# lorenzsp/EMRI_FrequencyDomainWaveforms

Hardware: AMD Instinct MI355X
Metric: FD waveforms/sec (2 yr, dt=10 s, ~3000 modes) at 1/2/4/8 GPUs; mode-sum HBM GB/s (higher is better)
Workload: dtype f64

## Files before the change

### emri_frequencydomainwaveforms_amd/csrc/emrifd.hip

```cpp

#include "emrifd_layout.h"

#define EFD_VERSION 100

static thread_local std::string g_err;

int efdhip::fail(int code, const std::string& msg) {
    g_err = msg;
    return code;
}

namespace {

constexpr int NWAVE = TILE / 64;
constexpr int XCD_GROUP = 1024 / TILE;
constexpr int SEGWIN = TILE;
constexpr int PIECES = (int)sizeof(Item) / 16;
constexpr int B_PIECE = (int)offsetof(Item, b) / 16;
constexpr int ROUNDS = 2;
constexpr int NC = (ROUNDS * TILE) / PIECES;


__device__ __forceinline__ bool seg_hits_tile(int2 lh, int32_t tlo, int32_t thi) {
    return lh.y > tlo && lh.x < thi;
// ... 1063 lines not shown
#pragma clang fp contract(off)
                    const int64_t q = j - k0, nb = nf - k0;
                    const double2 d0 = reinterpret_cast<const double2*>(lld)[q];
                    const double2 d1 = reinterpret_cast<const double2*>(lld)[nb + q];
                    const double w0 = llw[q], w1 = llw[nb + q];
                    const double r0 = d0.x - vp.x * w0, i0 = d0.y - vp.y * w0;
                    const double r1 = d1.x - vc.x * w1, i1 = d1.y - vc.y * w1;
                    llacc = fma(r0, r0, fma(i0, i0, llacc));
                    llacc = fma(r1, r1, fma(i1, i1, llacc));
                }
                if (!php) return;
                if (accumulate_out) {
                    const double2 pp = php[j - k0], pc = phc[j - k0];
                    vp.x += pp.x; vp.y += pp.y; vc.x += pc.x; vc.y += pc.y;
                }
                php[j - k0] = vp;
                phc[j - k0] = vc;
            };
            put(km, sm, sk);
            if (km != k) put(k, sk, sm);
        }
    }
    if constexpr (EPI == EPI_DH) {
        if (PAIRED && lld) {
            __shared__ double dhw4[3][NWAVE];
#pragma unroll
            for (int s = 0; s < 3; ++s) {
#pragma unroll
                for (int o = 32; o > 0; o >>= 1) dh[s] += __shfl_xor(dh[s], o, 64);
                if (lane == 0) dhw4[s][wave] = dh[s];
            }
            __syncthreads();
            if (tid < 3) {
                double t = 0.0;
#pragma unroll
                for (int w = 0; w < NWAVE; ++w) t += dhw4[tid][w];
                llpart[tid * ntiles + tile] = t;
            }
        }
    } else if (PAIRED && lld) {
#pragma unroll
        for (int o = 32; o > 0; o >>= 1) llacc += __shfl_xor(llacc, o, 64);
        __shared__ double llw4[NWAVE];
        if (lane == 0) llw4[wave] = llacc;
        __syncthreads();
        if (tid == 0) {
            double t = 0.0;
#pragma unroll
            for (int w = 0; w < NWAVE; ++w) t += llw4[w];
            llpart[tile] = t;
        }
    }
}

struct SumDesc {
    const Item* items;
    const int4* ranges;
    const int2* seglh;
    const int4* seginfo;
    const int32_t* nseg;
    const double* freq;
    const int32_t* gm;
    const int32_t* gn;
    const double* t;
    const double* coefA;
    const double* coefT;
    const double2* sctab;
    const uint32_t* tkeys;
    const int32_t* tcnt;
    const int32_t* tperm;
    const int32_t* segbase;
    const int32_t* stb0;
    const int32_t* stb1;
    Header* hdr;
    double* out;
    double* hp;
    double* hc;
    double* llpart;
    int64_t k0;
    int32_t nt, K;
};
template <bool PAIRED, int CAUSTIC, int NB = BPL, int EPI = EPI_LL>
__device__ __forceinline__ void modesum_tile(
    const SumDesc d, int64_t nf, int64_t nlanes, int64_t ntiles, int accumulate_out,
    const double* __restrict__ lld, const double* __restrict__ llw,
    const double* __restrict__ llconst, int64_t b, bool direct = false, int ioff = 0,
    double* __restrict__ spart = nullptr, int32_t* __restrict__ scnt = nullptr) {
    modesum_tile<PAIRED, CAUSTIC, NB, EPI>(
        d.items, d.ranges, d.seglh, d.seginfo, d.nseg, d.freq, nf, nlanes, ntiles, d.nt, d.K,
        d.gm, d.gn, d.t, d.coefA, d.coefT, d.sctab, d.tkeys, d.tcnt, d.tperm, d.segbase, d.stb0,
        d.stb1, d.hdr, accumulate_out, d.out, d.hp, d.hc, d.k0, lld, llw, d.llpart, llconst, b,
        direct, ioff, spart, scnt);
}

template <bool PAIRED, int CAUSTIC, int BPL>
__global__ __launch_bounds__(TILE) __attribute__((amdgpu_waves_per_eu(EFD_WAVES_PER_EU, 8)))
void k_modesum(const SumDesc d, int64_t nf, int64_t nlanes, int64_t ntiles, int accumulate_out) {
    modesum_tile<PAIRED, CAUSTIC>(d, nf, nlanes, ntiles, accumulate_out, nullptr, nullptr,
                                  nullptr, (int64_t)blockIdx.x);
}

struct SumBatch {
    SumDesc d[EFD_BATCH_MAX];
    int32_t n;
};
static_assert(sizeof(SumBatch) <= 3584, "batch descriptors must fit the kernel arguments");
template <class Outside>
__device__ __forceinline__ void ll_final_reduce(const double* __restrict__ p,
                                                const Header* __restrict__ h, bool sparse,
                                                Outside outside, int64_t ntiles, double scale,
                                                double* __restrict__ out) {
    __shared__ double red[256];
    int64_t t0 = 0, t1 = ntiles - 1;
    if (sparse) {
        const int32_t lo = h->lane_lo, hi = h->lane_hi;
        t0 = lo < hi ? lo / TILE_LANES : ntiles;
        t1 = lo < hi ? (int64_t)(hi - 1) / TILE_LANES : -1;
    }
    auto val = [&](int64_t i) { return (i < t0 || i > t1) ? outside(i) : p[i]; };
    double acc = 0.0;
    int64_t i = threadIdx.x;
    for (; i + 3 * 256 < ntiles; i += 4 * 256) {
        const double v0 = val(i), v1 = val(i + 256), v2 = val(i + 512), v3 = val(i + 768);
        acc += v0;
        acc += v1;
        acc += v2;
        acc += v3;
    }
    for (; i < ntiles; i += 256) acc += val(i);
    red[threadIdx.x] = acc;
    __syncthreads();
    for (int s = 128; s > 0; s >>= 1) {
        if ((int)threadIdx.x < s) red[threadIdx.x] += red[threadIdx.x + s];
        __syncthreads();
    }
    if (threadIdx.x == 0) {
        const bool bad = h->runs_overflow | h->bad_mn | h->bad_tile;
        *out = bad ? __longlong_as_double(0x7ff8000000000000LL) : scale * red[0];
    }
}
template <bool PAIRED, int CAUSTIC, int BPL, bool SPARSE, int EPI = EPI_LL>
__global__ __launch_bounds__(TILE) __attribute__((amdgpu_waves_per_eu(EFD_WAVES_PER_EU, 8)))
void k_modesum_batch(const SumBatch batch, int64_t nf, int64_t nlanes, int64_t ntiles,
                     int accumulate_out, const double* __restrict__ lld,
                     const double* __restrict__ llw, const double* __restrict__ llconst,
                     int64_t nper) {
    const int n = batch.n;
    int w;
    int64_t pos;
    if (lld == nullptr) {
        w = (int)(blockIdx.x % (unsigned)n);
        pos = blockIdx.x / (unsigned)n;
    } else {
        const unsigned g = blockIdx.x, r = g >> 3;
        w = (int)(r % (unsigned)n);
        pos = (int64_t)(r / (unsigned)n) * 8 + (g & 7u);
    }
    const SumDesc& d = batch.d[w];
    if constexpr (SPARSE) {
        const int32_t nit = d.hdr->nitems;
        if (nit > 0) {
            const Layout L = make_layout(d.nt, d.K, nf, 1);
            char* W = reinterpret_cast<char*>(d.hdr);
            const int4* items = ws_at<const int4>(W, L.sitem);
            for (int64_t it = pos; it < nit; it += nper) {
                const int4 e = items[it];
                const int S = e.y & 0xffff, j = e.y >> 16;
                if (S > 1)
                    modesum_tile<PAIRED, CAUSTIC, 1, EPI>(
                        d, nf, nlanes, ntiles, accumulate_out, lld, llw, llconst, e.x, true, j,
                        ws_at<double>(W, L.spart) + (size_t)e.z * TILE_LANES * 4,
                        ws_at<int32_t>(W, L.scnt) + e.w);
                else
                    modesum_tile<PAIRED, CAUSTIC, BPL, EPI>(d, nf, nlanes, ntiles, accumulate_out,
                                                            lld, llw, llconst, e.x, true);
                __syncthreads();
            }
            return;
        }
        const int32_t lo = d.hdr->lane_lo, hi = d.hdr->lane_hi;
        if (lo < hi) {
            const int64_t t1 = min((int64_t)(hi - 1) / TILE_LANES, ntiles - 1);
            for (int64_t tile = lo / TILE_LANES + pos; tile <= t1; tile += nper) {
                modesum_tile<PAIRED, CAUSTIC, BPL, EPI>(d, nf, nlanes, ntiles, accumulate_out, lld,
                                                        llw, llconst, tile, true);
                __syncthreads();
            }
        }
        return;
    }
    modesum_tile<PAIRED, CAUSTIC, BPL, EPI>(d, nf, nlanes, ntiles, accumulate_out, lld, llw,
                                            llconst, pos);
}

template <int BPL>
__global__ __launch_bounds__(TILE) void k_ll_tile_const(const double* __restrict__ lld,
                                                        const double* __restrict__ llw,
                                                        int64_t nf, int64_t nlanes, int64_t k0,
                                                        double* __restrict__ llconst) {
    const int64_t tile = blockIdx.x;
    __builtin_amdgcn_s_setreg(1 | (6 << 6) | (1 << 11), 0);
    __builtin_amdgcn_s_setreg(1 | (9 << 6), 0);
    const int tid = threadIdx.x;
    const int lane = tid & 63;
    const int wave = __builtin_amdgcn_readfirstlane(tid >> 6);
    const int32_t w_lo = (int32_t)(tile * TILE_LANES + wave * 64 * BPL);
    double llacc = 0.0;
#pragma unroll
    for (int i = 0; i < BPL; ++i) {
        const int64_t k = w_lo + 64 * i + lane;
        if (k >= nlanes) continue;
        const int64_t km = nf - 1 - k;
        double2 sk = make_double2(0.0, 0.0);
        double2 sm = make_double2(0.0, 0.0);
        if (km == k) {
            sk.x += sm.x;
            sk.y += sm.y;
            sm = sk;
        }
        auto put = [&](int64_t j, double2 a, double2 b) {
            if (j < k0) return;
            double2 vp = make_double2(0.5 * (a.x + b.x), 0.5 * (a.y - b.y));
            double2 vc = make_double2(-0.5 * (a.y + b.y), 0.5 * (a.x - b.x));
            {
#pragma clang fp contract(off)
                const int64_t q = j - k0, nb = nf - k0;
                const double2 d0 = reinterpret_cast<const double2*>(lld)[q];
                const double2 d1 = reinterpret_cast<const double2*>(lld)[nb + q];
                const double w0 = llw[q], w1 = llw[nb + q];
                const double r0 = d0.x - vp.x * w0, i0 = d0.y - vp.y * w0;
                const double r1 = d1.x - vc.x * w1, i1 = d1.y - vc.y * w1;
                llacc = fma(r0, r0, fma(i0, i0, llacc));
                llacc = fma(r1, r1, fma(i1, i1, llacc));
            }
        };
        put(km, sm, sk);
        if (km != k) put(k, sk, sm);
    }
#pragma unroll
    for (int o = 32; o > 0; o >>= 1) llacc += __shfl_xor(llacc, o, 64);
    __shared__ double llw4[NWAVE];
    if (lane == 0) llw4[wave] = llacc;
    __syncthreads();
    if (tid == 0) {
        double t = 0.0;
#pragma unroll
        for (int w = 0; w < NWAVE; ++w) t += llw4[w];
        llconst[tile] = t;
    }
}

struct LlBatch {
    const double* part[EFD_BATCH_MAX];
    const Header* hdr[EFD_BATCH_MAX];
    double* out;
    const double* llconst;
    int64_t ntiles;
    int32_t n;
};
struct StatusBatch {
    Header* h[EFD_BATCH_MAX];
    int32_t n;
};
__global__ __launch_bounds__(64) void k_lane_gather(const StatusBatch sb, int32_t* out) {
    const int i = threadIdx.x;
    if (i >= sb.n) return;
    out[2 * i] = sb.h[i]->lane_lo;
    out[2 * i + 1] = sb.h[i]->lane_hi;
}
__global__ __launch_bounds__(64) void k_status_gather(const StatusBatch sb, int32_t* out) {
    const int i = threadIdx.x;
    if (i >= sb.n) return;
    Header* h = sb.h[i];
    const int32_t f = (h->runs_overflow ? 1 : 0) | (h->bad_mn ? 2 : 0) | (h->bad_tile ? 4 : 0);
    out[i] = f;
    if (f) {
        h->runs_overflow = 0;
        h->bad_mn = 0;
        h->bad_tile = 0;
    }
}

__global__ __launch_bounds__(256) void k_ll_final(const LlBatch lb) {
    const double* llconst = lb.llconst;
    ll_final_reduce(lb.part[blockIdx.x], lb.hdr[blockIdx.x], llconst != nullptr,
                    [=](int64_t i) { return llconst[i]; }, lb.ntiles, -0.5 * 4.0,
                    lb.out + blockIdx.x);
}

struct DhBatch {
    const Header* hdr[EFD_BATCH_MAX];
    const double* part;
    double* out;
    int64_t ntiles;
    int32_t sparse;
};
__global__ __launch_bounds__(256) void k_dh_final(const DhBatch db) {
    const int64_t o = 3 * (int64_t)blockIdx.x + blockIdx.y;
    ll_final_reduce(db.part + o * db.ntiles, db.hdr[blockIdx.x], db.sparse != 0,
                    [](int64_t) { return 0.0; }, db.ntiles, 4.0, db.out + o);
}

constexpr int TK_HITS = TILE;
constexpr int TK_ROWS = 8;
__device__ __forceinline__ void tile_keys_body(
    const int4* __restrict__ ranges, const int2* __restrict__ seglh,
    const int4* __restrict__ seginfo, const int32_t* __restrict__ nsegp,
    const int32_t* __restrict__ segbase, const int32_t* __restrict__ stb0,
    const int32_t* __restrict__ stb1, int64_t ntiles, uint32_t* __restrict__ tkeys,
    int32_t* __restrict__ tcnt) {
    static_assert(SEGWIN == TILE, "one segment per thread and window row");
    __shared__ int hits[TK_HITS], hp0[TK_HITS], hcnt[TK_HITS], hoff[TK_HITS], hws[TK_HITS],
        hwt[TK_HITS];
    __shared__ int4 hinfo[TK_HITS];
    __shared__ int wcnt[TK_ROWS * NWAVE];
    __shared__ int part[NWAVE];
    const int64_t tile = blockIdx.x;
    if (tile >= ntiles) return;
    const int tid = threadIdx.x, lane = tid & 63;
    const int wave = __builtin_amdgcn_readfirstlane(tid >> 6);
    const int32_t tlo = (int32_t)(tile * TILE_LANES), thi = tlo + TILE_LANES;
    const int nseg = *nsegp;
    EFD_EXP_DO(if (tile == 0 && tid == 0) exp_add(27, (unsigned long long)nseg);)
    int nhit = 0;
    for (int base = 0; base < nseg; base += TK_ROWS * TILE) {
        unsigned long long bal[TK_ROWS];
#pragma unroll
        for (int r = 0; r < TK_ROWS; ++r) {
            const int sgi = base + r * TILE + tid;
            bool hit = false;
            if (sgi < nseg) hit = seg_hits_tile(seglh[sgi], tlo, thi);
            bal[r] = __ballot(hit);
            if (lane == 0) wcnt[r * NWAVE + wave] = __popcll(bal[r]);
        }
        __syncthreads();
#pragma unroll
        for (int r = 0; r < TK_ROWS; ++r) {
            int before = nhit;
            for (int w = 0; w < wave; ++w) before += wcnt[r * NWAVE + w];
            if ((bal[r] >> lane) & 1ull) {
                const int pos = before + __popcll(bal[r] & ((1ull << lane) - 1ull));
                if (pos < TK_HITS) hits[pos] = base + r * TILE + tid;
            }
#pragma unroll
            for (int w = 0; w < NWAVE; ++w) nhit += wcnt[r * NWAVE + w];
        }
        __syncthreads();
    }
    EFD_EXP_DO(if (tid == 0) exp_add(28, (unsigned long long)nhit);)
    if (nhit > TK_HITS) {
        if (tid == 0) tcnt[tile] = -1;
        return;
    }
    int c = 0;
    if (tid < nhit) {
        const int sg = hits[tid];
        const HitRecords hr = hit_records(sg, tile, tlo, thi, segbase, stb0, stb1, seginfo, ranges);
        c = hr.count;
        hp0[tid] = hr.p0;
        hcnt[tid] = c;
        hinfo[tid] = seginfo[sg];
    }
    int total;
    const int off = block_excl_scan<NWAVE>(c, part, lane, wave, total);
    if (total > KEYCAP) {
        if (tid == 0) tcnt[tile] = -1;
        return;
    }
    if (tid < nhit) hoff[tid] = off;
    __syncthreads();
    {
        const int w = tid < nhit ? hits[tid] / SEGWIN : INT32_MAX;
        const bool first = tid < nhit && (tid == 0 || hits[tid - 1] / SEGWIN != w);
        const bool last = tid < nhit && (tid == nhit - 1 || hits[tid + 1] / SEGWIN != w);
        int st = first ? off : INT32_MIN;
        int en = last ? off + c : INT32_MAX;
#pragma unroll
        for (int o = 1; o < 64; o <<= 1) {
            const int vs = __shfl_up(st, o, 64), ve = __shfl_down(en, o, 64);
            if (lane >= o) st = max(st, vs);
            if (lane + o < 64) en = min(en, ve);
        }
        if (lane == 63) hws[wave] = st;
        if (lane == 0) hwt[wave] = en;
        __syncthreads();
        for (int v = 0; v < wave; ++v) st = max(st, hws[v]);
        for (int v = NWAVE - 1; v > wave; --v) en = min(en, hwt[v]);
        __syncthreads();
        if (tid < nhit) {
            hws[tid] = st;
            hwt[tid] = en - st;
        }
    }
    __syncthreads();
    uint32_t* out = tkeys + (size_t)tile * KEYCAP;
    for (int g = tid; g < total; g += TILE) {
        int lo = 0, hi = nhit - 1;
        while (lo < hi) {
            const int mid = (lo + hi + 1) >> 1;
            if (hoff[mid] <= g) lo = mid; else hi = mid - 1;
        }
        const int ws = hws[lo], take = hwt[lo];
        out[ws + scatter_slot(g - ws, take)] = list_key(hinfo[lo], hp0[lo] + (g - hoff[lo]));
    }
    if (tid == 0) tcnt[tile] = total;
}
__global__ __launch_bounds__(TILE) void k_tile_keys(const PrepBatch B) {
    PREP_WALKER(B);
    if (D.lists == 0) return;
    tile_keys_body(ws_at<int4>(W, L.ranges), ws_at<int2>(W, L.seglh), ws_at<int4>(W, L.seginfo),
                   ws_at<int32_t>(W, L.nseg), ws_at<int32_t>(W, L.segbase),
                   ws_at<int32_t>(W, L.stb0), ws_at<int32_t>(W, L.stb1), L.ntiles,
                   ws_at<uint32_t>(W, L.tkeys), ws_at<int32_t>(W, L.tcnt));
}

constexpr int ORDER_BUCKETS = 64;
__device__ __forceinline__ int tile_cost_bucket(int32_t c) {
    if (c < 0) return ORDER_BUCKETS - 1;
    const float l = __log2f((float)c + 1.0f) * 4.0f;
    return min((int)l, ORDER_BUCKETS - 2);
}
__device__ __forceinline__ int wave_bucket_add(int* hist, int bucket, bool valid) {
    const int lane = threadIdx.x & 63;
    unsigned long long todo = __ballot(valid);
    int res = 0;
    while (todo) {
        const int leader = __ffsll((long long)todo) - 1;
        const int bl = __shfl(bucket, leader, 64);
        const unsigned long long same = __ballot(valid && bucket == bl) & todo;
        int base = 0;
        if (lane == leader) base = atomicAdd(&hist[bl], __popcll(same));
        base = __shfl(base, leader, 64);
        if ((same >> lane) & 1ull) res = base + __popcll(same & ((1ull << lane) - 1ull));
        todo &= ~same;
    }
    return res;
}
__device__ __forceinline__ void tile_order_body(const int32_t* __restrict__ tcnt,
                                                int64_t ntiles, int32_t* __restrict__ tperm) {
    __shared__ int hist[ORDER_BUCKETS];
    const int tid = threadIdx.x;
    if (tid < ORDER_BUCKETS) hist[tid] = 0;
    __syncthreads();
    constexpr int PER = 16;
    int bk[PER];
#pragma unroll
    for (int q = 0; q < PER; ++q) {
        const int64_t i = tid + (int64_t)q * 1024;
        bk[q] = i < ntiles ? tile_cost_bucket(tcnt[i]) : -1;
    }
#pragma unroll
    for (int q = 0; q < PER; ++q) wave_bucket_add(hist, bk[q], bk[q] >= 0);
    const int64_t npass = (ntiles + 1023) / 1024;
    for (int64_t p = PER; p < npass; ++p) {
        const int64_t i = tid + p * 1024;
        const int bkt = i < ntiles ? tile_cost_bucket(tcnt[i]) : 0;
        wave_bucket_add(hist, bkt, i < ntiles);
    }
    __syncthreads();
    if (tid == 0) {
        int acc = 0;
        for (int q = ORDER_BUCKETS - 1; q >= 0; --q) { const int h = hist[q]; hist[q] = acc; acc += h; }
    }
    __syncthreads();
#pragma unroll
    for (int q = 0; q < PER; ++q) {
        const int pos = wave_bucket_add(hist, bk[q], bk[q] >= 0);
        if (bk[q] >= 0) tperm[pos] = (int32_t)(tid + q * 1024);
    }
    for (int64_t p = PER; p < npass; ++p) {
        const int64_t i = tid + p * 1024;
        const int bkt = i < ntiles ? tile_cost_bucket(tcnt[i]) : 0;
        const int pos = wave_bucket_add(hist, bkt, i < ntiles);
        if (i < ntiles) tperm[pos] = (int32_t)i;
    }
}
__global__ __launch_bounds__(1024) void k_tile_order(const PrepBatch B) {
    PREP_WALKER(B);
    if (D.lists != 3) return;
    tile_order_body(ws_at<int32_t>(W, L.tcnt), L.ntiles, ws_at<int32_t>(W, L.tperm));
}

constexpr int TD_THREADS = 256;
constexpr int TD_SPL = 4;

__device__ __forceinline__ int knot_interval(const double* __restrict__ t, int nt, double x) {
    int lo = 0, hi = nt - 1;
    while (hi - lo > 1) {
        const int mid = (lo + hi) >> 1;
        if (t[mid] <= x) lo = mid; else hi = mid;
    }
    return lo;
}

template <bool WIN>
__global__ __launch_bounds__(TD_THREADS) void k_td_modesum(
    const double* __restrict__ t, int nt, const double* __restrict__ coefT,
    const double* __restrict__ coefA, const int32_t* __restrict__ gm,
    const int32_t* __restrict__ gn, int K, const Header* __restrict__ hdr, double dt,
    int64_t ns, int accumulate_out, double* __restrict__ out, double* __restrict__ hp,
    double* __restrict__ hc, const double* __restrict__ window) {
    const int64_t s_base = (int64_t)blockIdx.x * (TD_THREADS * TD_SPL) + threadIdx.x;
    const double t_end = t[nt - 1];
    const int G = hdr->groups;
    double w[TD_SPL], pphi[TD_SPL], pr[TD_SPL], zr[TD_SPL], zi[TD_SPL];
    int jj[TD_SPL];
    bool valid[TD_SPL];
    bool any_valid = false;
#pragma unroll
    for (int i = 0; i < TD_SPL; ++i) {
        const int64_t s = s_base + (int64_t)i * TD_THREADS;
        const double ts = (double)s * dt;
        valid[i] = s < ns && ts <= t_end;
        any_valid |= valid[i];
        jj[i] = valid[i] ? knot_interval(t, nt, ts) : nt - 2;
        w[i] = valid[i] ? ts - t[jj[i]] : 0.0;
        const double* ct = coefT + (size_t)jj[i] * 32;
        pphi[i] = fma(fma(fma(ct[0], w[i], ct[8]), w[i], ct[16]), w[i], ct[24]);
        pr[i] = fma(fma(fma(ct[1], w[i], ct[9]), w[i], ct[17]), w[i], ct[25]);
        double sn, cs;
        sincos_big(pr[i], sn, cs);
        zr[i] = cs;
        zi[i] = -sn;
    }
    double Hr[TD_SPL], Hi[TD_SPL];
#pragma unroll
    for (int i = 0; i < TD_SPL; ++i) Hr[i] = Hi[i] = 0.0;

    if (__any(any_valid) && G > 0) {
        const int j0 = (int)rfl((uint32_t)jj[0]);
        bool same = true;
#pragma unroll
        for (int i = 0; i < TD_SPL; ++i) same &= jj[i] == j0;
        const size_t row = (size_t)4 * 4 * K;
        auto run = [&](auto UNI) {
            constexpr bool U = decltype(UNI)::value;
            double Pr[TD_SPL], Pi[TD_SPL], Qr[TD_SPL], Qi[TD_SPL];
#pragma unroll
            for (int i = 0; i < TD_SPL; ++i) Pr[i] = Pi[i] = Qr[i] = Qi[i] = 0.0;
            auto flush = [&](int m, int n0) {
#pragma unroll
                for (int i = 0; i < TD_SPL; ++i) {
                    double sn, cs;
                    sincos_big(fma((double)m, pphi[i], (double)n0 * pr[i]), sn, cs);
                    const double br = cs, bi = -sn;
                    Hr[i] += (br * Pr[i] - bi * Pi[i]) + (br * Qr[i] - bi * Qi[i]);
                    Hi[i] += (br * Pi[i] + bi * Pr[i]) - (br * Qi[i] + bi * Qr[i]);
                    Pr[i] = Pi[i] = Qr[i] = Qi[i] = 0.0;
                }
            };
            int cur_m = gm[G - 1], nprev = gn[G - 1];
            for (int g = G - 1; g >= 0; --g) {
                const int m = gm[g], n = gn[g];
                int d = nprev - n;
                if (m != cur_m) {
                    flush(cur_m, nprev);
                    cur_m = m;
                    d = 1;
                }
                nprev = n;
                for (; d > 1; --d) {
#pragma unroll
                    for (int i = 0; i < TD_SPL; ++i) {
                        const double a = Pr[i], b = Qr[i];
                        Pr[i] = fma(a, zr[i], -Pi[i] * zi[i]);
                        Pi[i] = fma(a, zi[i], Pi[i] * zr[i]);
                        Qr[i] = fma(b, zr[i], -Qi[i] * zi[i]);
                        Qi[i] = fma(b, zi[i], Qi[i] * zr[i]);
                    }
                }
#pragma unroll
                for (int i = 0; i < TD_SPL; ++i) {
                    const double* ca = coefA + (size_t)(U ? j0 : jj[i]) * row + 4 * g;
                    const double wi = w[i];
                    const double bpr = fma(fma(fma(ca[0], wi, ca[4 * K]), wi, ca[8 * K]), wi, ca[12 * K]);
                    const double bpi = fma(fma(fma(ca[1], wi, ca[4 * K + 1]), wi, ca[8 * K + 1]), wi, ca[12 * K + 1]);
                    const double bmr = fma(fma(fma(ca[2], wi, ca[4 * K + 2]), wi, ca[8 * K + 2]), wi, ca[12 * K + 2]);
                    const double bmi = fma(fma(fma(ca[3], wi, ca[4 * K + 3]), wi, ca[8 * K + 3]), wi, ca[12 * K + 3]);
                    const double a = Pr[i], b = Qr[i];
                    Pr[i] = fma(a, zr[i], fma(-Pi[i], zi[i], bpr));
                    Pi[i] = fma(a, zi[i], fma(Pi[i], zr[i], bpi));
                    Qr[i] = fma(b, zr[i], fma(-Qi[i], zi[i], bmr));
                    Qi[i] = fma(b, zi[i], fma(Qi[i], zr[i], bmi));
                }
            }
            flush(cur_m, nprev);
        };
        if (__all(same)) run(std::integral_constant<bool, true>{});
        else run(std::integral_constant<bool, false>{});
    }

    double2* o = reinterpret_cast<double2*>(out);
#pragma unroll
    for (int i = 0; i < TD_SPL; ++i) {
        const int64_t s = s_base + (int64_t)i * TD_THREADS;
        if (s >= ns) continue;
        double vr = valid[i] ? -Hr[i] : 0.0, vi = valid[i] ? -Hi[i] : 0.0;
        if constexpr (WIN) {
            const double wv = window[s];
            vr *= wv;
            vi *= wv;
        }
        if (o) {
            double2 v = make_double2(vr, vi);
            if (accumulate_out) { const double2 p = o[s]; v.x += p.x; v.y += p.y; }
            o[s] = v;
        }
        if (hp) hp[s] = accumulate_out ? hp[s] + vr : vr;
        if (hc) hc[s] = accumulate_out ? hc[s] - vi : -vi;
    }
}

}


static int64_t resident_tile_slots() {
    constexpr int MAX_DEV = 64;
    static std::atomic<int64_t> cache[MAX_DEV];
    int dev = 0;
    if (hipGetDevice(&dev) != hipSuccess || dev < 0 || dev >= MAX_DEV) return 1024;
    int64_t v = cache[dev].load(std::memory_order_relaxed);
    if (v > 0) return v;
    int cus = 0, per_cu = 0;
    if (hipDeviceGetAttribute(&cus, hipDeviceAttributeMultiprocessorCount, dev) != hipSuccess ||
        hipOccupancyMaxActiveBlocksPerMultiprocessor(
            &per_cu, reinterpret_cast<const void*>(&k_modesum<true, EFD_CAUSTIC_UNIFORM, BPL>),
            TILE, 0) != hipSuccess || cus <= 0 || per_cu <= 0)
        return 1024;
    v = (int64_t)cus * per_cu;
    cache[dev].store(v, std::memory_order_relaxed);
    return v;
}

constexpr int32_t ORDER_MIN_K = 1024;
constexpr int32_t LISTS_MIN_K = 1024;
static int32_t lists_min_k() {
    static const int32_t v = [] {
        const char* e = std::getenv("EFD_LISTS_MIN_K");
        return e ? (int32_t)std::atoi(e) : LISTS_MIN_K;
    }();
    return v;
}
static bool use_prebuilt(int32_t K) { return K >= lists_min_k(); }
static bool use_cost_order(int64_t ntiles, int32_t K) {
    return use_prebuilt(K) && K >= ORDER_MIN_K && ntiles > resident_tile_slots();
}
int32_t efdhip::list_mode(int32_t K, int64_t ntiles) {
    return use_prebuilt(K) ? (use_cost_order(ntiles, K) ? 3 : 1) : 0;
}

int efdhip::check_modesum_args(const efd_modesum_args* a, const void* workspace, int phase) {
    if (!a || !workspace) return fail(EFD_ERR_ARG, "efd_modesum: NULL argument");
    if (!a->t || !a->phi_phi || !a->phi_r || !a->f_phi || !a->f_r || !a->amp || !a->m ||
        !a->n || !a->ylm_p || !a->ylm_m || !a->freq)
        return fail(EFD_ERR_ARG, "efd_modesum: NULL array");
    const bool pol = a->hp != nullptr || a->hc != nullptr;
    if (pol && (!a->hp || !a->hc || !a->grid_symmetric || a->k0 < 0 || a->k0 > a->nf))
        return fail(EFD_ERR_ARG, "efd_modesum: hp/hc need both pointers, a symmetric grid and "
                                 "0 <= k0 <= nf");
    if ((phase & 2) && !a->out && !pol)
        return fail(EFD_ERR_ARG, "efd_modesum: no output (out or hp/hc)");
    if (a->nt < 2 || a->nt > MAX_NT) return fail(EFD_ERR_ARG, "efd_modesum: nt out of range");
    if (a->K <= 0 || a->K > MAX_K) return fail(EFD_ERR_ARG, "efd_modesum: K out of range [1, 8192]");
    if (a->nf <= 0 || a->nf >= (int64_t)INT32_MAX)
        return fail(EFD_ERR_ARG, "efd_modesum: nf out of range");
    if (a->caustic != EFD_CAUSTIC_SPA && a->caustic != EFD_CAUSTIC_UNIFORM)
        return fail(EFD_ERR_ARG, "efd_modesum: unknown caustic mode");
    return EFD_OK;
}

int efdhip::launch_tile_lists(const void* prep_batch, int64_t ntiles, bool any_lists,
                              bool any_order, hipStream_t st) {
    const PrepBatch& B = *static_cast<const PrepBatch*>(prep_batch);
    const unsigned nz = (unsigned)B.n;
    if (any_lists) {
        hipLaunchKernelGGL(k_tile_keys, dim3((unsigned)ntiles, 1, nz), dim3(TILE), 0, st, B);
        HIP_TRY(hipGetLastError());
    }
    if (any_order) {
        hipLaunchKernelGGL(k_tile_order, dim3(1, 1, nz), dim3(1024), 0, st, B);
        HIP_TRY(hipGetLastError());
    }
    return EFD_OK;
}

static SumDesc sum_desc(const efd_modesum_args* a, void* workspace, const Layout& L) {
    char* ws = (char*)workspace;
    const int32_t lists = efdhip::list_mode(a->K, L.ntiles);
    SumDesc d{};
    d.items = (const Item*)(ws + L.items);
    d.ranges = (const int4*)(ws + L.ranges);
    d.seglh = (const int2*)(ws + L.seglh);
    d.seginfo = (const int4*)(ws + L.seginfo);
    d.nseg = (const int32_t*)(ws + L.nseg);
    d.freq = a->freq;
    d.gm = (const int32_t*)(ws + L.gm);
    d.gn = (const int32_t*)(ws + L.gn);
    d.t = a->t;
    d.coefA = (const double*)(ws + L.coefA);
    d.coefT = (const double*)(ws + L.coefT);
    d.sctab = (const double2*)(ws + L.sctab);
    d.tkeys = (const uint32_t*)(ws + L.tkeys);
    d.tcnt = lists ? (const int32_t*)(ws + L.tcnt) : nullptr;
    d.tperm = lists == 3 ? (const int32_t*)(ws + L.tperm) : nullptr;
    d.segbase = (const int32_t*)(ws + L.segbase);
    d.stb0 = (const int32_t*)(ws + L.stb0);
    d.stb1 = (const int32_t*)(ws + L.stb1);
    d.hdr = (Header*)(ws + L.header);
    d.out = a->out;
    d.hp = a->hp;
    d.hc = a->hc;
    d.llpart = (double*)(ws + L.llpart);
    d.k0 = a->k0;
    d.nt = a->nt;
    d.K = a->K;
    return d;
}

template <class F>
static void for_sum_variant(bool paired, int caustic, F f) {
    using Uniform = std::integral_constant<int, EFD_CAUSTIC_UNIFORM>;
    using Spa = std::integral_constant<int, EFD_CAUSTIC_SPA>;
    if (paired) {
        if (caustic == EFD_CAUSTIC_UNIFORM) f(std::true_type{}, Uniform{});
        else f(std::true_type{}, Spa{});
    } else {
        if (caustic == EFD_CAUSTIC_UNIFORM) f(std::false_type{}, Uniform{});
        else f(std::false_type{}, Spa{});
    }
}

static int read_header(const void* workspace, void* stream, Header& h) {
    HIP_TRY(hipStreamSynchronize((hipStream_t)stream));
    HIP_TRY(hipMemcpy(&h, workspace, sizeof(Header), hipMemcpyDeviceToHost));
    return EFD_OK;
}

static int fill_status_batch(const char* fn, void* const* workspace, int32_t count,
                             StatusBatch& sb) {
    sb.n = count;
    for (int i = 0; i < count; ++i) {
        if (!workspace[i]) return fail(EFD_ERR_ARG, std::string(fn) + ": NULL workspace");
        sb.h[i] = (Header*)workspace[i];
    }
    return EFD_OK;
}

static int status_error(int32_t flags, const std::string& who) {
    if (flags & 1) return fail(EFD_ERR_ARG, who + "a harmonic has more than 8 monotonic runs");
    if (flags & 2) return fail(EFD_ERR_ARG, who + "|m| > 255 or |n| > 1023");
    return fail(EFD_ERR_HIP, who + "a tile dispatch-order entry was out of range (prepare/sum "
                                   "workspace mismatch?); bins were left unwritten");
}

extern "C" {

int efd_version(void) { return EFD_VERSION; }

#ifndef EFD_BUILD_ID
#define EFD_BUILD_ID "unversioned"
#endif
__attribute__((used)) static const char efd_build_tag[] = "EFD_BUILD_ID=" EFD_BUILD_ID;
const char* efd_build_id(void) { return efd_build_tag + 13; }

#ifdef EFD_EXP
int efd_exp_counters(unsigned long long* out) {
    HIP_TRY(hipDeviceSynchronize());
    HIP_TRY(hipMemcpyFromSymbol(out, HIP_SYMBOL(g_exp_count), sizeof(unsigned long long) * EXP_NCOUNT));
    return EFD_OK;
}
int efd_exp_tiles(unsigned int* out, unsigned long long* clk) {
    HIP_TRY(hipDeviceSynchronize());
    HIP_TRY(hipMemcpyFromSymbol(out, HIP_SYMBOL(g_exp_tile), sizeof(unsigned int) * 16384));
    HIP_TRY(hipMemcpyFromSymbol(clk, HIP_SYMBOL(g_exp_tclk), sizeof(unsigned long long) * 16384));
    return EFD_OK;
}
#endif

int efd_last_error(char* buf, int len) {
    if (!buf || len <= 0) return EFD_ERR_ARG;
    std::snprintf(buf, (size_t)len, "%s", g_err.c_str());
    return EFD_OK;
}

size_t efd_modesum_workspace_bytes(int32_t nt, int32_t K, int64_t nf) {
    if (nt < 2 || nt > MAX_NT || K <= 0 || K > MAX_K || nf <= 0) return 0;
    return make_layout(nt, K, nf, 0).total;
}

static int modesum_impl(const efd_modesum_args* a, void* workspace, size_t workspace_bytes,
                        void* stream, int phase) {
    {
        const int rc = efdhip::check_modesum_args(a, workspace, phase);
        if (rc != EFD_OK) return rc;
    }
    const int paired = a->grid_symmetric ? 1 : 0;
    const Layout L = make_layout(a->nt, a->K, a->nf, paired);
    if (workspace_bytes < L.total)
        return fail(EFD_ERR_WORKSPACE, "efd_modesum: workspace too small (see efd_modesum_workspace_bytes)");

    hipStream_t st = (hipStream_t)stream;
    if (phase & 1) {
        const int rc = efdhip::prepare_batch("efd_modesum_prepare", &a, &workspace,
                                             &workspace_bytes, 1, stream);
        if (rc != EFD_OK) return rc;
    }
    if (phase & 2) {
        const int64_t gq = 8 * XCD_GROUP;
        const dim3 grid((unsigned)((L.ntiles + gq - 1) / gq * gq)), block(TILE);
        const int acc = a->accumulate ? 1 : 0;
        const SumDesc d = sum_desc(a, workspace, L);
        if (a->prof_begin) HIP_TRY(hipEventRecord((hipEvent_t)a->prof_begin, st));
        for_sum_variant(paired != 0, a->caustic, [&](auto P, auto C) {
            hipLaunchKernelGGL((k_modesum<decltype(P)::value, decltype(C)::value, BPL>), grid,
                               block, 0, st, d, a->nf, L.nlanes, L.ntiles, acc);
        });
        HIP_TRY(hipGetLastError());
        if (a->prof_end) HIP_TRY(hipEventRecord((hipEvent_t)a->prof_end, st));
    }
    return EFD_OK;
}

int efd_modesum(const efd_modesum_args* a, void* workspace, size_t workspace_bytes, void* stream) {
    return modesum_impl(a, workspace, workspace_bytes, stream, 3);
}

int efd_modesum_sum(const efd_modesum_args* a, void* workspace, size_t workspace_bytes,
                    void* stream) {
    return modesum_impl(a, workspace, workspace_bytes, stream, 2);
}

constexpr int64_t SPARSE_WG = 4096;
static int64_t sparse_wg() {
    static const int64_t v = [] {
        const char* e = getenv("EFD_SPARSE_WG");
        const long long x = e ? atoll(e) : 0;
        return x >= 64 && x <= (1 << 20) ? (int64_t)x : SPARSE_WG;
    }();
    return v;
}
int sum_batch_impl(const char* fn, const efd_modesum_args* const* a, void* const* workspace,
                   const size_t* workspace_bytes, int32_t count, const double* d, const double* w,
                   double* llout, void* stream, const double* llconst = nullptr,
                   double* dhpart = nullptr, int32_t dhflags = 0) {
    const std::string F(fn);
    if (!a || !workspace || !workspace_bytes)
        return fail(EFD_ERR_ARG, F + ": NULL argument");
    if (count < 1 || count > EFD_BATCH_MAX)
        return fail(EFD_ERR_ARG, F + ": count out of range [1, EFD_BATCH_MAX]");
    SumBatch batch{};
    batch.n = count;
    Layout L0{};
    for (int i = 0; i < count; ++i) {
        const efd_modesum_args* ai = a[i];
        const int rc = efdhip::check_modesum_args(ai, workspace[i], d ? 0 : 2);
        if (rc != EFD_OK) return rc;
        if (ai->nf != a[0]->nf || (ai->grid_symmetric != 0) != (a[0]->grid_symmetric != 0) ||
            ai->caustic != a[0]->caustic || (ai->accumulate != 0) != (a[0]->accumulate != 0))
            return fail(EFD_ERR_ARG, F + ": nf, grid_symmetric, caustic and accumulate must agree "
                                         "across the batch");
        if (d && (!ai->grid_symmetric || ai->accumulate || ai->k0 != a[0]->k0 || ai->k0 < 0 ||
                  ai->k0 >= ai->nf))
            return fail(EFD_ERR_ARG, F + ": the fused likelihood needs a symmetric grid, "
                                         "accumulate = 0 and one 0 <= k0 < nf for the batch");
        const int paired = ai->grid_symmetric ? 1 : 0;
        const Layout L = make_layout(ai->nt, ai->K, ai->nf, paired);
        if (workspace_bytes[i] < L.total)
            return fail(EFD_ERR_WORKSPACE, F + ": workspace too small (see "
                                               "efd_modesum_workspace_bytes)");
        if (i == 0) L0 = L;
        batch.d[i] = sum_desc(ai, workspace[i], L);
        if (dhpart) batch.d[i].llpart = dhpart + (size_t)i * 3 * L.ntiles;
    }
    hipStream_t st = (hipStream_t)stream;
    bool sparse = d != nullptr && (dhpart ? !(dhflags & 1) : llconst != nullptr) &&
                  a[0]->grid_symmetric;
    for (int i = 0; i < count && sparse; ++i)
        sparse = !a[i]->out && !a[i]->hp && !a[i]->hc &&
                 efdhip::list_mode(a[i]->K, L0.ntiles) == 0;
    const int64_t gq = 8 * XCD_GROUP;
    int64_t nper = 0;
    if (sparse) {
        const int64_t cap = std::max<int64_t>(64, (sparse_wg() / count + 7) / 8 * 8);
        bool planned = true;
        for (int i = 0; i < count; ++i) planned = planned && a[i]->K <= SEG1_MAX_K;
        nper = planned ? cap : std::min<int64_t>((L0.ntiles + 7) / 8 * 8, cap);
    }
    const int64_t nblk = sparse ? nper * count : (L0.ntiles + gq - 1) / gq * gq * count;
    if (nblk > (int64_t)UINT32_MAX) return fail(EFD_ERR_ARG, F + ": grid too large");
    const dim3 grid((unsigned)nblk), block(TILE);
    const int acc = a[0]->accumulate ? 1 : 0;
    if (a[0]->prof_begin) HIP_TRY(hipEventRecord((hipEvent_t)a[0]->prof_begin, st));
    for_sum_variant(a[0]->grid_symmetric != 0, a[0]->caustic, [&](auto P, auto C) {
        constexpr bool PAIRED = decltype(P)::value;
        constexpr int CAUSTIC = decltype(C)::value;
        if constexpr (PAIRED) {
            if (dhpart) {
                if (sparse)
                    hipLaunchKernelGGL((k_modesum_batch<true, CAUSTIC, BPL, true, EPI_DH>), grid,
                                       block, 0, st, batch, a[0]->nf, L0.nlanes, L0.ntiles, acc, d,
                                       w, nullptr, nper);
                else
                    hipLaunchKernelGGL((k_modesum_batch<true, CAUSTIC, BPL, false, EPI_DH>), grid,
                                       block, 0, st, batch, a[0]->nf, L0.nlanes, L0.ntiles, acc, d,
                                       w, nullptr, (int64_t)0);
                return;
            }
        }
        if (sparse)
            hipLaunchKernelGGL((k_modesum_batch<PAIRED, CAUSTIC, BPL, true>), grid, block, 0, st,
                               batch, a[0]->nf, L0.nlanes, L0.ntiles, acc, d, w, llconst, nper);
        else
            hipLaunchKernelGGL((k_modesum_batch<PAIRED, CAUSTIC, BPL, false>), grid, block, 0, st,
                               batch, a[0]->nf, L0.nlanes, L0.ntiles, acc, d, w,
                               d ? llconst : nullptr, (int64_t)0);
    });
    HIP_TRY(hipGetLastError());
    if (dhpart) {
        DhBatch db{};
        for (int i = 0; i < count; ++i) db.hdr[i] = (const Header*)workspace[i];
        db.part = dhpart;
        db.out = llout;
        db.ntiles = L0.ntiles;
        db.sparse = sparse ? 1 : 0;
        hipLaunchKernelGGL(k_dh_final, dim3((unsigned)count, 3), dim3(256), 0, st, db);
        HIP_TRY(hipGetLastError());
    } else if (d) {
        LlBatch lb{};
        lb.n = count;
        lb.ntiles = L0.ntiles;
        for (int i = 0; i < count; ++i) {
            lb.part[i] = batch.d[i].llpart;
            lb.hdr[i] = (const Header*)workspace[i];
        }
        lb.out = llout;
        lb.llconst = sparse ? llconst : nullptr;
        hipLaunchKernelGGL(k_ll_final, dim3((unsigned)count), dim3(256), 0, st, lb);
        HIP_TRY(hipGetLastError());
    }
    if (a[0]->prof_end) HIP_TRY(hipEventRecord((hipEvent_t)a[0]->prof_end, st));
    return EFD_OK;
}

int efd_modesum_sum_batch(const efd_modesum_args* const* a, void* const* workspace,
                          const size_t* workspace_bytes, int32_t count, void* stream) {
    return sum_batch_impl("efd_modesum_sum_batch", a, workspace, workspace_bytes, count, nullptr,
                          nullptr, nullptr, stream);
}

int efd_modesum_sum_loglike(const efd_modesum_args* const* a, void* const* workspace,
                            const size_t* workspace_bytes, int32_t count, const double* d,
                            const double* w, double* out, void* stream) {
    if (!d || !w || !out) return fail(EFD_ERR_ARG, "efd_modesum_sum_loglike: NULL d, w or out");
    return sum_batch_impl("efd_modesum_sum_loglike", a, workspace, workspace_bytes, count, d, w,
                          out, stream);
}

int efd_modesum_sum_dh_hh(const efd_modesum_args* const* a, void* const* workspace,
                          const size_t* workspace_bytes, int32_t count, const double* d,
                          const double* w, double* part, int32_t flags, double* out,
                          void* stream) {
    if (!d || !w || !part || !out)
        return fail(EFD_ERR_ARG, "efd_modesum_sum_dh_hh: NULL d, w, part or out");
    return sum_batch_impl("efd_modesum_sum_dh_hh", a, workspace, workspace_bytes, count, d, w, out,
                          stream, nullptr, part, flags);
}

int64_t efd_loglike_tile_count(int64_t nf) {
    if (nf < 1) return 0;
    return make_layout(2, 1, nf, 1).ntiles;
}

int efd_loglike_tile_constants(const double* d, const double* w, int64_t nf, int64_t k0,
                               double* tile_const, void* stream) {
    if (!d || !w || !tile_const)
        return fail(EFD_ERR_ARG, "efd_loglike_tile_constants: NULL d, w or tile_const");
    if (nf < 1 || k0 < 0 || k0 >= nf)
        return fail(EFD_ERR_ARG, "efd_loglike_tile_constants: need nf >= 1 and 0 <= k0 < nf");
    const Layout L = make_layout(2, 1, nf, 1);
// ... 234 lines not shown
```

Measured before the change: 1953.

## Assign one tile per wavefront in tile-key construction, dropping block barriers

The tile-key kernel now processes one tile per 64-lane wavefront instead of one tile per block. Hit collection, the count scan, and the window start/end scans become purely wave-local using ballots and shuffles, with per-wave LDS slices. The block-wide __syncthreads and cross-wave counters are removed, and the grid shrinks by NWAVE. Each lane now handles several hit rounds, and shared memory per block grows, which could lower occupancy.

After: 1971 (median of 6 runs). Within noise of the previous version (+1.0%).

```diff
diff --git a/emri_frequencydomainwaveforms_amd/csrc/emrifd.hip b/emri_frequencydomainwaveforms_amd/csrc/emrifd.hip
--- a/emri_frequencydomainwaveforms_amd/csrc/emrifd.hip
+++ b/emri_frequencydomainwaveforms_amd/csrc/emrifd.hip
@@ -1389,108 +1389,143 @@
 }
 
 constexpr int TK_HITS = TILE;
-constexpr int TK_ROWS = 8;
+constexpr int TK_ROUNDS = TK_HITS / 64;
+constexpr int TK_LOADS = 8;
+static_assert(TK_HITS % 64 == 0, "hits are taken in whole rounds of a wave");
+struct TkWave {
+    int hits[TK_HITS], hp0[TK_HITS], hoff[TK_HITS], hws[TK_HITS], hwt[TK_HITS];
+    int4 hinfo[TK_HITS];
+};
+__device__ __forceinline__ void tk_wave_sync() {
+    __builtin_amdgcn_fence(__ATOMIC_RELEASE, "wavefront");
+    __builtin_amdgcn_wave_barrier();
+    __builtin_amdgcn_fence(__ATOMIC_ACQUIRE, "wavefront");
+}
 __device__ __forceinline__ void tile_keys_body(
     const int4* __restrict__ ranges, const int2* __restrict__ seglh,
     const int4* __restrict__ seginfo, const int32_t* __restrict__ nsegp,
     const int32_t* __restrict__ segbase, const int32_t* __restrict__ stb0,
     const int32_t* __restrict__ stb1, int64_t ntiles, uint32_t* __restrict__ tkeys,
     int32_t* __restrict__ tcnt) {
-    static_assert(SEGWIN == TILE, "one segment per thread and window row");
-    __shared__ int hits[TK_HITS], hp0[TK_HITS], hcnt[TK_HITS], hoff[TK_HITS], hws[TK_HITS],
-        hwt[TK_HITS];
-    __shared__ int4 hinfo[TK_HITS];
-    __shared__ int wcnt[TK_ROWS * NWAVE];
-    __shared__ int part[NWAVE];
-    const int64_t tile = blockIdx.x;
+    __shared__ TkWave slice[NWAVE];
+    const int lane = threadIdx.x & 63;
+    const int wave = __builtin_amdgcn_readfirstlane(threadIdx.x >> 6);
+    const int64_t tile = (int64_t)NWAVE * blockIdx.x + wave;
     if (tile >= ntiles) return;
-    const int tid = threadIdx.x, lane = tid & 63;
-    const int wave = __builtin_amdgcn_readfirstlane(tid >> 6);
+    TkWave& S = slice[wave];
+    const unsigned long long below = (1ull << lane) - 1ull;
     const int32_t tlo = (int32_t)(tile * TILE_LANES), thi = tlo + TILE_LANES;
     const int nseg = *nsegp;
-    EFD_EXP_DO(if (tile == 0 && tid == 0) exp_add(27, (unsigned long long)nseg);)
+    EFD_EXP_DO(if (tile == 0 && lane == 0) exp_add(27, (unsigned long long)nseg);)
     int nhit = 0;
-    for (int base = 0; base < nseg; base += TK_ROWS * TILE) {
-        unsigned long long bal[TK_ROWS];
-#pragma unroll
-        for (int r = 0; r < TK_ROWS; ++r) {
-            const int sgi = base + r * TILE + tid;
-            bool hit = false;
-            if (sgi < nseg) hit = seg_hits_tile(seglh[sgi], tlo, thi);
-            bal[r] = __ballot(hit);
-            if (lane == 0) wcnt[r * NWAVE + wave] = __popcll(bal[r]);
-        }
-        __syncthreads();
-#pragma unroll
-        for (int r = 0; r < TK_ROWS; ++r) {
-            int before = nhit;
-            for (int w = 0; w < wave; ++w) before += wcnt[r * NWAVE + w];
-            if ((bal[r] >> lane) & 1ull) {
-                const int pos = before + __popcll(bal[r] & ((1ull << lane) - 1ull));
-                if (pos < TK_HITS) hits[pos] = base + r * TILE + tid;
+    for (int base = 0; base < nseg; base += TK_LOADS * 64) {
+        bool hit[TK_LOADS];
+#pragma unroll
+        for (int r = 0; r < TK_LOADS; ++r) {
+            const int sgi = base + r * 64 + lane;
+            hit[r] = sgi < nseg && seg_hits_tile(seglh[sgi], tlo, thi);
+        }
+#pragma unroll
+        for (int r = 0; r < TK_LOADS; ++r) {
+            const unsigned long long bal = __ballot(hit[r]);
+            if (hit[r]) {
+                const int pos = nhit + __popcll(bal & below);
+                if (pos < TK_HITS) S.hits[pos] = base + r * 64 + lane;
             }
-#pragma unroll
-            for (int w = 0; w < NWAVE; ++w) nhit += wcnt[r * NWAVE + w];
-        }
-        __syncthreads();
-    }
-    EFD_EXP_DO(if (tid == 0) exp_add(28, (unsigned long long)nhit);)
-    if (nhit > TK_HITS) {
-        if (tid == 0) tcnt[tile] = -1;
+            nhit += __popcll(bal);
+        }
+    }
+    EFD_EXP_DO(if (lane == 0) exp_add(28, (unsigned long long)nhit);)
+    if (nhit == 0 || nhit > TK_HITS) {
+        if (lane == 0) tcnt[tile] = nhit == 0 ? 0 : -1;
         return;
     }
-    int c = 0;
-    if (tid < nhit) {
-        const int sg = hits[tid];
-        const HitRecords hr = hit_records(sg, tile, tlo, thi, segbase, stb0, stb1, seginfo, ranges);
-        c = hr.count;
-        hp0[tid] = hr.p0;
-        hcnt[tid] = c;
-        hinfo[tid] = seginfo[sg];
-    }
-    int total;
-    const int off = block_excl_scan<NWAVE>(c, part, lane, wave, total);
+    tk_wave_sync();
+    int sgs[TK_ROUNDS], cs[TK_ROUNDS], offs[TK_ROUNDS];
+#pragma unroll
+    for (int r = 0; r < TK_ROUNDS; ++r) {
+        const int i = r * 64 + lane;
+        sgs[r] = -1;
+        cs[r] = 0;
+        if (i < nhit) {
+            const int sg = S.hits[i];
+            const HitRecords hr =
+                hit_records(sg, tile, tlo, thi, segbase, stb0, stb1, seginfo, ranges);
+            sgs[r] = sg;
+            cs[r] = hr.count;
+            S.hp0[i] = hr.p0;
+            S.hinfo[i] = seginfo[sg];
+        }
+    }
+    int total = 0;
+#pragma unroll
+    for (int r = 0; r < TK_ROUNDS; ++r) {
+        int incl = cs[r];
+#pragma unroll
+        for (int o = 1; o < 64; o <<= 1) {
+            const int u = __shfl_up(incl, o, 64);
+            if (lane >= o) incl += u;
+        }
+        offs[r] = total + incl - cs[r];
+        total += __shfl(incl, 63, 64);
+    }
     if (total > KEYCAP) {
-        if (tid == 0) tcnt[tile] = -1;
+        if (lane == 0) tcnt[tile] = -1;
         return;
     }
-    if (tid < nhit) hoff[tid] = off;
-    __syncthreads();
+    int sts[TK_ROUNDS], ens[TK_ROUNDS];
+#pragma unroll
+    for (int r = 0; r < TK_ROUNDS; ++r) {
+        const int i = r * 64 + lane;
+        const bool in = i < nhit;
+        const int w = in ? sgs[r] / SEGWIN : INT32_MAX;
+        const bool first = in && (i == 0 || S.hits[i - 1] / SEGWIN != w);
+        const bool last = in && (i == nhit - 1 || S.hits[i + 1] / SEGWIN != w);
+        sts[r] = first ? offs[r] : INT32_MIN;
+        ens[r] = last ? offs[r] + cs[r] : INT32_MAX;
+#pragma unroll
+        for (int o = 1; o < 64; o <<= 1) {
+            const int vs = __shfl_up(sts[r], o, 64), ve = __shfl_down(ens[r], o, 64);
+            if (lane >= o) sts[r] = max(sts[r], vs);
+            if (lane + o < 64) ens[r] = min(ens[r], ve);
+        }
+    }
     {
-        const int w = tid < nhit ? hits[tid] / SEGWIN : INT32_MAX;
-        const bool first = tid < nhit && (tid == 0 || hits[tid - 1] / SEGWIN != w);
-        const bool last = tid < nhit && (tid == nhit - 1 || hits[tid + 1] / SEGWIN != w);
-        int st = first ? off : INT32_MIN;
-        int en = last ? off + c : INT32_MAX;
-#pragma unroll
-        for (int o = 1; o < 64; o <<= 1) {
-            const int vs = __shfl_up(st, o, 64), ve = __shfl_down(en, o, 64);
-            if (lane >= o) st = max(st, vs);
-            if (lane + o < 64) en = min(en, ve);
-        }
-        if (lane == 63) hws[wave] = st;
-        if (lane == 0) hwt[wave] = en;
-        __syncthreads();
-        for (int v = 0; v < wave; ++v) st = max(st, hws[v]);
-        for (int v = NWAVE - 1; v > wave; --v) en = min(en, hwt[v]);
-        __syncthreads();
-        if (tid < nhit) {
-            hws[tid] = st;
-            hwt[tid] = en - st;
-        }
-    }
-    __syncthreads();
+        int carry = INT32_MIN;
+#pragma unroll
+        for (int r = 0; r < TK_ROUNDS; ++r) {
+            sts[r] = max(sts[r], carry);
+            carry = __shfl(sts[r], 63, 64);
+        }
+        carry = INT32_MAX;
+#pragma unroll
+        for (int r = TK_ROUNDS - 1; r >= 0; --r) {
+            ens[r] = min(ens[r], carry);
+            carry = __shfl(ens[r], 0, 64);
+        }
+    }
+#pragma unroll
+    for (int r = 0; r < TK_ROUNDS; ++r) {
+        const int i = r * 64 + lane;
+        if (i < nhit) {
+            S.hoff[i] = offs[r];
+            S.hws[i] = sts[r];
+            S.hwt[i] = ens[r] - sts[r];
+        }
+    }
+    tk_wave_sync();
     uint32_t* out = tkeys + (size_t)tile * KEYCAP;
-    for (int g = tid; g < total; g += TILE) {
+    for (int g = lane; g < total; g += 64) {
         int lo = 0, hi = nhit - 1;
         while (lo < hi) {
             const int mid = (lo + hi + 1) >> 1;
-            if (hoff[mid] <= g) lo = mid; else hi = mid - 1;
-        }
-        const int ws = hws[lo], take = hwt[lo];
-        out[ws + scatter_slot(g - ws, take)] = list_key(hinfo[lo], hp0[lo] + (g - hoff[lo]));
-    }
-    if (tid == 0) tcnt[tile] = total;
+            if (S.hoff[mid] <= g) lo = mid; else hi = mid - 1;
+        }
+        const int ws = S.hws[lo], take = S.hwt[lo];
+        out[ws + scatter_slot(g - ws, take)] =
+            list_key(S.hinfo[lo], S.hp0[lo] + (g - S.hoff[lo]));
+    }
+    if (lane == 0) tcnt[tile] = total;
 }
 __global__ __launch_bounds__(TILE) void k_tile_keys(const PrepBatch B) {
     PREP_WALKER(B);
@@ -1761,7 +1796,8 @@
     const PrepBatch& B = *static_cast<const PrepBatch*>(prep_batch);
     const unsigned nz = (unsigned)B.n;
     if (any_lists) {
-        hipLaunchKernelGGL(k_tile_keys, dim3((unsigned)ntiles, 1, nz), dim3(TILE), 0, st, B);
+        hipLaunchKernelGGL(k_tile_keys, dim3((unsigned)((ntiles + NWAVE - 1) / NWAVE), 1, nz),
+                           dim3(TILE), 0, st, B);
         HIP_TRY(hipGetLastError());
     }
     if (any_order) {
```
